# jkw0701/closed_chain_motion_planner

Hardware: AMD Instinct MI355X
Metric: constraint projections/sec (dual-Panda Wine_Bottle) (higher is better)
Workload: dtype f64

## Files before the change

### closed_chain_motion_planner_amd/build.py

```python
import os
import shutil
import subprocess

HERE = os.path.dirname(os.path.abspath(__file__))
CSRC = os.path.join(HERE, "csrc")
LIBDIR = os.path.join(HERE, "lib")
LIBPATH = os.environ.get("CCMP_LIBRARY") or os.path.join(LIBDIR, "libccmp.so")
DEBUG_LIBPATH = os.path.join(LIBDIR, "libccmp_debug.so")
_DEBUG_UNITS = ("ccmp_api.cpp", "ccmp_policy.cpp")
_DEBUG_ONLY_UNITS = [("ccmp_kernels_debug.hip", ["-O3", "-ffp-contract=off", "-DCCMP_USE_FMA", "-DCCMP_LEAN_SQRT", "-DCCMP_LEAN_DIV", "-mllvm", "-disable-machine-licm"])]
ARCH = "gfx950"

_UNITS = [
    ("ccmp_kernels_fd.hip", ["-O3", "-ffp-contract=off", "-DCCMP_USE_FMA", "-DCCMP_LEAN_SQRT", "-DCCMP_ATAN_UNIFORM", "-DCCMP_FD_TI_HOIST",
                             "-mllvm", "-disable-machine-licm", "-mllvm", "-amdgpu-sched-strategy=max-ilp"]
     + os.environ.get("CCMP_FD_EXTRA_FLAGS", "").split()),
    ("ccmp_kernels_wave.hip", ["-O3", "-ffp-contract=off", "-DCCMP_USE_FMA"]),
    ("ccmp_kernels_flat.hip", ["-O3", "-ffp-contract=off", "-DCCMP_USE_FMA", "-mllvm", "-disable-machine-licm", "-mllvm", "-amdgpu-sched-strategy=max-ilp"]),
    ("ccmp_kernels_geo.hip", ["-O3", "-ffp-contract=off", "-DCCMP_USE_FMA", "-mllvm", "-disable-machine-licm", "-mllvm", "-amdgpu-sched-strategy=max-ilp"]),
    ("ccmp_kernels_geo.hip", ["-O3", "-ffp-contract=off", "-DCCMP_USE_FMA", "-DCCMP_GEO_LATENCY", "-DCCMP_SUMS_IN_LANE", "-DCCMP_FLAT_MIN_WAVES=2", "-mllvm", "-amdgpu-sched-strategy=max-ilp"],
     "ccmp_kernels_geo_lat.hip.o"),
    ("ccmp_kernels_geo_scene.hip", ["-O3", "-ffp-contract=off", "-DCCMP_USE_FMA", "-DCCMP_SUMS_IN_LANE", "-DCCMP_FLAT_MIN_WAVES=2", "-mllvm", "-amdgpu-sched-strategy=max-ilp"]),
    ("ccmp_kernels_resident.hip", ["-O3", "-ffp-contract=off", "-DCCMP_USE_FMA", "-DCCMP_SUMS_IN_LANE", "-DCCMP_FLAT_MIN_WAVES=2", "-mllvm", "-amdgpu-sched-strategy=max-ilp"]),
    ("ccmp_kernels_fast.hip", ["-O3", "-ffp-contract=off", "-DCCMP_USE_FMA", "-DCCMP_LEAN_SQRT", "-mllvm", "-disable-machine-licm"]),
    ("ccmp_kernels_scout.hip", ["-O3", "-ffp-contract=fast", "-ffast-math", "-fno-slp-vectorize"]),
    ("ccmp_problem.cpp", ["-O2", "-ffp-contract=off", "-DCCMP_USE_FMA", "-x", "hip"]),
    ("ccmp_api.cpp", ["-O2", "-ffp-contract=off", "-DCCMP_USE_FMA", "-x", "hip"]),
    ("ccmp_policy.cpp", ["-O2", "-x", "hip"]),
    ("ccmp_resident.cpp", ["-O2", "-x", "hip"]),
    ("ccmp_host_io.cpp", ["-O2", "-x", "hip"]),
    ("ccmp_comm.cpp", ["-O2", "-x", "hip"]),
    ("ccmp_kernels_scene.hip", ["-O3", "-ffp-contract=off", "-DCCMP_USE_FMA", "-DCCMP_LEAN_SQRT"]),
    ("ccmp_scene.cpp", ["-O2", "-ffp-contract=off", "-DCCMP_USE_FMA", "-x", "hip"]),
]
_HEADERS = ["ccmp_detmath.h", "ccmp_kin.h", "ccmp_solve.h", "ccmp_fd_common.h", "ccmp_flat_newton.h", "ccmp_host.h", "ccmp_ctx.h", "ccmp_launch.h", "ccmp_policy.h", "ccmp_resident.h", "ccmp_fd_newton_phase1.inc", "ccmp_fd_newton_phase2.inc", "ccmp_geo_edge.h", "ccmp_geo_edge_body.inc", "ccmp_scene.h", "ccmp_clearance.h", "ccmp_row16_eval.inc", "ccmp_row16_step.inc", "ccmp_row16_geo_body.inc", os.path.join("..", "..", "include", "ccmp.h")]


def hipcc_path():
    for cand in (shutil.which("hipcc"), "/opt/rocm/bin/hipcc"):
        if cand and os.path.exists(cand):
            return cand
    raise RuntimeError("hipcc not found: libccmp.so cannot be built (no CPU fallback exists)")


def _stale(target, sources):
    if not os.path.exists(target):
        return True
    t = os.path.getmtime(target)
    return any(os.path.getmtime(s) > t for s in sources if os.path.exists(s))


_SCRATCH_RULES = [
    (r"(project_fd_kernel|project_fd_flat_kernel|project_fd_wave_kernel|geodesic_flat_kernel(_lat)?|geodesic_scene_kernel|geodesic_group_kernel|resident_service_kernel)<(\d+, )?true>", 0),
    (r"(project_fd_kernel|project_fd_flat_kernel|project_fd_wave_kernel|geodesic_flat_kernel(_lat)?|geodesic_scene_kernel|geodesic_group_kernel|resident_service_kernel)<(\d+, )?false>", 136),
    (r"project_pair_kernel|project_row16_kernel", 0),
    (r"geodesic_row16_(scene_)?kernel", 0),
    (r"scout_|clearance", 400),
    (r".", 64),
]


def _demangle(names):
    for tool in ("/opt/rocm/lib/llvm/bin/llvm-cxxfilt", shutil.which("c++filt")):
        if tool and os.path.exists(tool):
            out = subprocess.run([tool], input="\n".join(names), capture_output=True, text=True).stdout.split("\n")
            return dict(zip(names, out))
    return {n: n for n in names}


def parse_resource_remarks(stderr_text):
    import re

    kernels, cur = [], None
    keys = {"TotalSGPRs": "sgprs", "VGPRs": "vgprs", "AGPRs": "agprs", "ScratchSize [bytes/lane]": "scratch", "Occupancy [waves/SIMD]": "occupancy",
            "SGPRs Spill": "sgpr_spill", "VGPRs Spill": "vgpr_spill", "LDS Size [bytes/block]": "lds"}
    for line in stderr_text.splitlines():
        m = re.search(r"remark: (?:\s*)([A-Za-z \[\]/]+): (\S+) \[-Rpass-analysis", line)
        if not m:
            continue
        k, v = m.group(1).strip(), m.group(2)
        if k == "Function Name":
            cur = {"mangled": v}
            kernels.append(cur)
        elif cur is not None and k in keys:
            cur[keys[k]] = int(v)
    dm = _demangle([k["mangled"] for k in kernels])
    for k in kernels:
        k["name"] = dm[k["mangled"]].replace("(anonymous namespace)::", "").split("(")[0].replace("void ", "")
    return kernels


def check_resources(kernels, unit):
    import re

    bad = []
    for k in kernels:
        bound = next(b for rx, b in _SCRATCH_RULES if re.search(rx, k["name"]))
        k["scratch_bound"] = bound
        if k.get("scratch", 0) > bound:
            bad.append("%s: %d B/lane of scratch (bound %d), %d VGPRs, %d spilled" % (k["name"], k["scratch"], bound, k.get("vgprs", -1), k.get("vgpr_spill", -1)))
    if bad and not os.environ.get("CCMP_ALLOW_SPILLS"):
        raise RuntimeError("register allocation of %s regressed (closed_chain_motion_planner_amd/build.py: _SCRATCH_RULES; CCMP_ALLOW_SPILLS=1 "
                           "builds anyway):\n  " % unit + "\n  ".join(bad))


def resource_report():
    import glob
    import json

    return {os.path.basename(f)[:-len(".resources.json")]: json.load(open(f)) for f in sorted(glob.glob(os.path.join(HERE, "build", "*.resources.json")))}


def build_library(force=False, verbose=False):
    os.makedirs(LIBDIR, exist_ok=True)
    objdir = os.path.join(HERE, "build")
    os.makedirs(objdir, exist_ok=True)
    hipcc = hipcc_path()
    headers = [os.path.join(CSRC, h) for h in _HEADERS]
    objs, dbg_objs, jobs = [], [], []
    relink = force
    for src, flags, *obj in _UNITS:
        sp = os.path.join(CSRC, src)
        op = os.path.join(objdir, obj[0] if obj else src + ".o")
        objs.append(op)
        variants = [(op, [])]
        if src in _DEBUG_UNITS:
            dp = os.path.join(objdir, src + ".dbg.o")
            dbg_objs.append(dp)
            variants.append((dp, ["-DCCMP_DEBUG_HOOKS"]))
        else:
            dbg_objs.append(op)
        for target, extra in variants:
            if force or _stale(target, [sp] + headers):
                jobs.append([hipcc, "--offload-arch=" + ARCH, "-fPIC", "-std=c++17"] + flags + extra +
                            (["-Rpass-analysis=kernel-resource-usage"] if src.endswith(".hip") else []) + ["-c", sp, "-o", target])
    for src, flags in _DEBUG_ONLY_UNITS:
        sp, op = os.path.join(CSRC, src), os.path.join(objdir, src + ".o")
        dbg_objs.append(op)
        if force or _stale(op, [sp] + headers):
            jobs.append([hipcc, "--offload-arch=" + ARCH, "-fPIC", "-std=c++17"] + flags + ["-Rpass-analysis=kernel-resource-usage", "-c", sp, "-o", op])
    if jobs:
        import json
        from concurrent.futures import ThreadPoolExecutor

        def run(cmd):
            if verbose:
                print(" ".join(cmd))
            r = subprocess.run(cmd, capture_output=True, text=True)
            rest = "\n".join(ln for ln in r.stderr.splitlines() if "-Rpass-analysis=kernel-resource-usage" not in ln)
            if rest.strip():
                print(rest)
            if r.returncode != 0:
                raise subprocess.CalledProcessError(r.returncode, cmd)
            if "-Rpass-analysis=kernel-resource-usage" in cmd:
                kernels = parse_resource_remarks(r.stderr)
                try:
                    check_resources(kernels, os.path.basename(cmd[-1]))
                except RuntimeError:
                    os.remove(cmd[-1])
                    raise
                json.dump(kernels, open(cmd[-1][:-2] + ".resources.json", "w"), indent=1)

        workers = max(1, min(len(jobs), int(os.environ.get("CCMP_BUILD_JOBS", "0")) or min(4, os.cpu_count() or 1)))
        with ThreadPoolExecutor(workers) as pool:
            list(pool.map(run, jobs))
        relink = True
    default_lib = os.path.join(LIBDIR, "libccmp.so")
    for target, members in ((default_lib, objs), (DEBUG_LIBPATH, dbg_objs)):
        if relink or _stale(target, members):
            cmd = [hipcc, "--offload-arch=" + ARCH, "-shared", "-fPIC", "-o", target] + members
            if verbose:
                print(" ".join(cmd))
            subprocess.run(cmd, check=True)
    return LIBPATH


if __name__ == "__main__":
    print(build_library(force=True, verbose=True))
```

### closed_chain_motion_planner_amd/csrc/ccmp_kernels_fd.hip

```cpp
#include <hip/hip_runtime.h>
#include <stdint.h>

#include "ccmp_fd_common.h"

using namespace ccmp;

namespace {

constexpr int kGroup = 6;
constexpr int kGroupsPerWave = 10;
constexpr int kX = 0;
constexpr int kSC = 14;
constexpr int kPre = 42;
constexpr int kEE = 126;
constexpr int kJ0 = 150;
constexpr int kRec = 165;

#ifndef CCMP_FD_WAVES_PER_SIMD
#define CCMP_FD_WAVES_PER_SIMD 3
#endif
#ifndef CCMP_FD_STOCK_COLUMNS
#define CCMP_FD_STOCK_COLUMNS 1
#endif
#ifndef CCMP_FD_ROWS
#define CCMP_FD_ROWS 1
#endif

template <int ARM, bool STORE, bool STOCK, int I>
__device__ __forceinline__ void chain_at_x_from(const ccmp_consts &K, double *rec, bool writer, double *R, double *o)
{
  if constexpr (I < 7) {
    double Rn[9];
    mulvec_acc_nz<STOCK ? kStockOff[I] : 7>(R, K.offset[ARM][I], o);
    if (STORE && writer) {
#pragma unroll
      for (int k = 0; k < 9; k++) rec[kPre + I * 12 + k] = R[k];
#pragma unroll
      for (int k = 0; k < 3; k++) rec[kPre + I * 12 + 9 + k] = o[k];
    }
    chain_rot<I, STOCK>(K.axis[ARM][I], K.aprod[ARM][I], rec[kSC + 2 * (ARM * 7 + I)], rec[kSC + 2 * (ARM * 7 + I) + 1], R, Rn);
#pragma unroll
    for (int k = 0; k < 9; k++) R[k] = Rn[k];
    chain_at_x_from<ARM, STORE, STOCK, I + 1>(K, rec, writer, R, o);
  }
}
template <int ARM, bool STORE, bool STOCK>
__device__ __forceinline__ void chain_at_x(const ccmp_consts &K, double *rec, bool writer, double *T)
{
  double R[9] = {1, 0, 0, 0, 1, 0, 0, 0, 1}, o[3] = {0, 0, 0};
  if constexpr (STOCK) {
    chain_at_x_from<ARM, STORE, true, 0>(K, rec, writer, R, o);
  } else {
    for (int i = 0; i < 7; i++) {
      double Rj[9], Rn[9];
      mulvec_acc(R, K.offset[ARM][i], o);
      if (STORE && writer) {
#pragma unroll
        for (int k = 0; k < 9; k++) rec[kPre + i * 12 + k] = R[k];
#pragma unroll
        for (int k = 0; k < 3; k++) rec[kPre + i * 12 + 9 + k] = o[k];
      }
      rot_sc(K.axis[ARM][i], K.aprod[ARM][i], rec[kSC + 2 * (ARM * 7 + i)], rec[kSC + 2 * (ARM * 7 + i) + 1], Rj);
      mul33(R, Rj, Rn);
#pragma unroll
      for (int k = 0; k < 9; k++) R[k] = Rn[k];
    }
  }
  tool_pose_t<STOCK>(K, ARM, R, o, &T[0], &T[9]);
}

template <bool TOOL, int I>
__device__ __forceinline__ void chain_rows_from(const ccmp_consts &K, double *rec, const double *sc, int row, bool store,
                                                double &R0, double &R1, double &R2, double &o)
{
  if constexpr (I < 7) {
    constexpr int NZ = kStockOff[I];
    if (NZ & 1) o = CCMP_FMA(R0, K.offset[0][I][0], o);
    if (NZ & 2) o = CCMP_FMA(R1, K.offset[0][I][1], o);
    if (NZ & 4) o = CCMP_FMA(R2, K.offset[0][I][2], o);
    if (store) {
      rec[kPre + I * 12 + 3 * row] = R0;
      rec[kPre + I * 12 + 3 * row + 1] = R1;
      rec[kPre + I * 12 + 3 * row + 2] = R2;
      rec[kPre + I * 12 + 9 + row] = o;
    }
    const double s = sc[2 * I], c = sc[2 * I + 1];
    double n0, n1, n2;
    if constexpr (kStockZ[I] != 0) {
      const double t = 1.0 - c;
      const double w = t + c;
      const double ns = -s;
      n0 = CCMP_FMA(R1, s, R0 * c);
      n1 = CCMP_FMA(R1, c, R0 * ns);
      n2 = R2 * w;
    } else {
      double Rj[9];
      rot_sc(K.axis[0][I], K.aprod[0][I], s, c, Rj);
      n0 = dot3(R0, Rj[0], R1, Rj[3], R2, Rj[6]);
      n1 = dot3(R0, Rj[1], R1, Rj[4], R2, Rj[7]);
      n2 = dot3(R0, Rj[2], R1, Rj[5], R2, Rj[8]);
    }
    R0 = n0; R1 = n1; R2 = n2;
    chain_rows_from<TOOL, I + 1>(K, rec, sc, row, store, R0, R1, R2, o);
  }
}
template <bool TOOL>
__device__ __forceinline__ void chain_rows(const ccmp_consts &K, double *rec, int arm, int row, bool live, int store_arm,
                                           double d_lane, double bp_lane)
{
  double R0 = row == 0 ? 1.0 : 0.0, R1 = row == 1 ? 1.0 : 0.0, R2 = row == 2 ? 1.0 : 0.0, o = 0.0;
  chain_rows_from<TOOL, 0>(K, rec, rec + kSC + 14 * arm, row, live && arm == store_arm, R0, R1, R2, o);
  if constexpr (TOOL) {
    double pf = o;
    if (kStockEe & 1) pf = CCMP_FMA(R0, K.ee[0][0], pf);
    if (kStockEe & 2) pf = CCMP_FMA(R1, K.ee[0][1], pf);
    if (kStockEe & 4) pf = CCMP_FMA(R2, K.ee[0][2], pf);
    const double *Rt = K.R_tool[0];
    const double f0 = dot3(R0, Rt[0], R1, Rt[3], R2, Rt[6]);
    const double f1 = dot3(R0, Rt[1], R1, Rt[4], R2, Rt[7]);
    const double f2 = dot3(R0, Rt[2], R1, Rt[5], R2, Rt[8]);
    if (live) {
      double *T = rec + kEE + 12 * arm;
      T[3 * row] = d_lane * f0;
      T[3 * row + 1] = d_lane * f1;
      T[3 * row + 2] = d_lane * f2;
      T[9 + row] = CCMP_FMA(d_lane, pf, bp_lane);
    }
  }
}

__device__ __forceinline__ void stock_z_step(const ccmp_consts &K, int i, double s, double c, const double *R, double *Rn, double *o)
{
  const double ox = K.offset[0][i][0], oz = K.offset[0][i][2];
#pragma unroll
  for (int r = 0; r < 3; r++) o[r] = CCMP_FMA(R[3 * r + 2], oz, CCMP_FMA(R[3 * r], ox, o[r]));
  mul_zrot(R, s, c, Rn);
}
__device__ __forceinline__ void stock_g_step(const ccmp_consts &K, int i, double s, double c, const double *R, double *Rn, double *o)
{
  const double ox = K.offset[0][i][0];
#pragma unroll
  for (int r = 0; r < 3; r++) o[r] = CCMP_FMA(R[3 * r], ox, o[r]);
  double Rj[9];
  rot_sc(K.axis[0][i], K.aprod[0][i], s, c, Rj);
  mul33(R, Rj, Rn);
}

template <int ARM, bool STOCK>
__device__ __forceinline__ void jacobian_columns(const ccmp_consts &K, double *rec, bool live, int r, bool plus, int nstep)
{
  double To[12];
#pragma unroll
  for (int k = 0; k < 12; k++) To[k] = rec[kEE + (1 - ARM) * 12 + k];
#ifdef CCMP_FD_TI_HOIST
  if (ARM == 0) {
    double ti[3];
    mulTvec(&To[0], &To[9], ti);
#pragma unroll
    for (int k = 0; k < 3; k++) To[9 + k] = ti[k];
  }
#endif
  for (int j = 0; j < 7; j++) {
    const double xj = rec[kX + ARM * 7 + j];
    const double axj = ccmp_abs(xj);
    const double h = 1.4901161193847656e-08 * (axj >= 1 ? axj : 1);
    const double hh = plus ? h : -h;
    double y = xj + hh;
    if (nstep >= 2) y = y + hh;
    if (nstep >= 3) y = y + hh;
    double R[9], o[3], s, c;
#pragma unroll
    for (int k = 0; k < 9; k++) R[k] = rec[kPre + j * 12 + k];
#pragma unroll
    for (int k = 0; k < 3; k++) o[k] = rec[kPre + j * 12 + 9 + k];
    ccmp_sincos(y, &s, &c);
    const double *sc = rec + kSC + 2 * ARM * 7;
    if constexpr (STOCK && CCMP_FD_STOCK_COLUMNS) {
      double Rn[9];
      int i = j + 1;
      if ((j & 1) == 0 && j < 6) {
        const double t = 1.0 - c;
        const double w = t + c;
        const double ns = -s;
#pragma unroll
        for (int rr = 0; rr < 3; rr++) {
          const double a = R[3 * rr], b = R[3 * rr + 1];
          R[3 * rr] = CCMP_FMA(b, s, a * c);
          R[3 * rr + 1] = CCMP_FMA(b, c, a * ns);
          R[3 * rr + 2] = R[3 * rr + 2] * w;
        }
      } else {
        double Rj[9];
        rot_sc(K.axis[0][j], K.aprod[0][j], s, c, Rj);
        mul33(R, Rj, Rn);
        if (j < 6) {
          if (i < 6) stock_z_step(K, i, sc[2 * i], sc[2 * i + 1], Rn, R, o);
          else stock_g_step(K, 6, sc[12], sc[13], Rn, R, o);
          i++;
        } else {
#pragma unroll
          for (int k = 0; k < 9; k++) R[k] = Rn[k];
        }
      }
      for (; i < 5; i += 2) {
        stock_g_step(K, i, sc[2 * i], sc[2 * i + 1], R, Rn, o);
        stock_z_step(K, i + 1, sc[2 * i + 2], sc[2 * i + 3], Rn, R, o);
      }
      if (i == 5) {
        double Rj[9];
        rot_sc(K.axis[0][5], K.aprod[0][5], sc[10], sc[11], Rj);
        mul33(R, Rj, Rn);
        stock_g_step(K, 6, sc[12], sc[13], Rn, R, o);
      }
    } else {
      {
        double Rj[9], Rn[9];
        rot_sc(K.axis[ARM][j], K.aprod[ARM][j], s, c, Rj);
        mul33(R, Rj, Rn);
#pragma unroll
        for (int k = 0; k < 9; k++) R[k] = Rn[k];
      }
      {
        int i = j + 1;
        if ((7 - i) & 1) {
          joint_step(K, ARM, i, sc[2 * i], sc[2 * i + 1], R, o);
          i++;
        }
        for (; i < 7; i += 2) {
          double Rj[9], Rn[9];
          mulvec_acc(R, K.offset[ARM][i], o);
          rot_sc(K.axis[ARM][i], K.aprod[ARM][i], sc[2 * i], sc[2 * i + 1], Rj);
          mul33(R, Rj, Rn);
          mulvec_acc(Rn, K.offset[ARM][i + 1], o);
          rot_sc(K.axis[ARM][i + 1], K.aprod[ARM][i + 1], sc[2 * i + 2], sc[2 * i + 3], Rj);
          mul33(Rn, Rj, R);
        }
      }
    }
#if defined(CCMP_FD_PROBE_MOV) || defined(CCMP_FD_PROBE_FMA)
    {
      int pv = j;
      double pa = xj, pb = xj;
#ifdef CCMP_FD_PROBE_MOV
#pragma unroll
      for (int k = 0; k < CCMP_FD_PROBE_MOV; k++) asm volatile("v_mov_b32 %0, 0x12345678" : "=v"(pv));
#endif
#ifdef CCMP_FD_PROBE_FMA
#pragma unroll
      for (int k = 0; k < CCMP_FD_PROBE_FMA / 2; k++) asm volatile("v_fma_f64 %0, %0, %2, %2\n v_fma_f64 %1, %1, %2, %2" : "+v"(pa), "+v"(pb) : "v"(h));
#endif
      if (pv == 0x7fffffff || pa + pb == 12345.678) rec[kX] = pa;
    }
#endif
    double Tw[12], t[2];
    tool_pose_t<STOCK>(K, ARM, R, o, &Tw[0], &Tw[9]);
#ifdef CCMP_FD_TI_HOIST
    if (ARM == 0) chain_residual_ti(K, &Tw[0], &Tw[9], &To[0], &To[9], t, nullptr, nullptr);
#else
    if (ARM == 0) chain_residual(K, &Tw[0], &Tw[9], &To[0], &To[9], t, nullptr, nullptr);
#endif
    else chain_residual(K, &To[0], &To[9], &Tw[0], &Tw[9], t, nullptr, nullptr);
    if (live) {
      rec[kPre + 12 * j + 2 * r] = t[0];
      rec[kPre + 12 * j + 2 * r + 1] = t[1];
    }
  }
}

template <int ARM>
__device__ __forceinline__ void stencil_combine(double *rec, int r, bool live)
{
#pragma unroll
  for (int n = 0; n < 3; n++) {
    const int e = r + kGroup * n;
    if (e < 14 && live) {
      const int c = e >> 1, row = e & 1;
      const double xj = rec[kX + ARM * 7 + c];
      const double axj = ccmp_abs(xj);
      const double h = 1.4901161193847656e-08 * (axj >= 1 ? axj : 1);
      double y1 = xj, y2 = xj, m[3];
#pragma unroll
      for (int sidx = 0; sidx < 3; sidx++) {
        y1 = y1 + h;
        y2 = y2 - h;
        m[sidx] = (rec[kPre + 12 * c + 2 * sidx + row] - rec[kPre + 12 * c + 2 * (sidx + 3) + row]) / (y1 - y2);
      }
      const double Jv = CCMP_FMA(0.1, m[2], CCMP_FMA(-0.6, m[1], 1.5 * m[0]));
      if (ARM == 0) rec[kJ0 + 2 * c + row] = Jv;
      else rec[kSC + 2 * c + row] = Jv;
    }
  }
}

template <int MODE, bool STOCK>
__global__ __launch_bounds__(64, CCMP_FD_WAVES_PER_SIMD) void project_fd_kernel(
    const ccmp_consts K, const double *__restrict__ q_in, double *__restrict__ q_out, uint8_t *__restrict__ ok_out,
    uint16_t *__restrict__ iters_out, double *__restrict__ q_ambient, unsigned long long B, unsigned long long *queue,
    unsigned long long seed, unsigned long long first_index, double *__restrict__ pool, unsigned long long *pool_count,
    int dump_threshold, const unsigned int *__restrict__ order, const uint16_t *__restrict__ pred, int long_remaining,
    unsigned long long pool_records)
{
  __shared__ double lds[kGroupsPerWave * kRec];
  const int lane = threadIdx.x;
  const int g = lane / kGroup;
  const int r = lane - kGroup * g;
  const bool live = g < kGroupsPerWave;
  const int leader = live ? kGroup * g : 0;
  double *rec = lds + (live ? g : 0) * kRec;
  const bool writer = live && r == 0;
  const bool plus = r < 3;
  const int nstep = (plus ? r : r - 3) + 1;
  const int arm_l = plus ? 0 : 1, row_l = plus ? r : r - 3;
  double d_lane = 0.0, bp_lane = 0.0;
  if constexpr (STOCK) {
    d_lane = arm_l ? (row_l == 0 ? K.base_R[1][0] : (row_l == 1 ? K.base_R[1][4] : K.base_R[1][8]))
                   : (row_l == 0 ? K.base_R[0][0] : (row_l == 1 ? K.base_R[0][4] : K.base_R[0][8]));
    bp_lane = arm_l ? (row_l == 0 ? K.base_p[1][0] : (row_l == 1 ? K.base_p[1][1] : K.base_p[1][2]))
                    : (row_l == 0 ? K.base_p[0][0] : (row_l == 1 ? K.base_p[0][1] : K.base_p[0][2]));
  }

  unsigned long long idx = 0;
  int iter = 0, updates = 0;
  double norm1 = 0.0, norm2 = 0.0;
  bool active = false, drained = false;

  for (;;) {
    {
      const bool want = live && !active && !drained;
      unsigned long long t = 0;
      if (want && r == 0) t = atomicAdd(queue, 1ull);
      t = shfl_u64(t, leader);
      if (want) {
        if (t < B) {
          idx = order ? (unsigned long long)order[t] : t;
          active = true; iter = 0; updates = 0; norm1 = 0.0; norm2 = 0.0;
          if (MODE == 0) {
            const double2 *row = reinterpret_cast<const double2 *>(q_in + idx * 14);
            const double2 a = row[r];
            rec[kX + 2 * r] = a.x;
            rec[kX + 2 * r + 1] = a.y;
            if (r == 0) {
              const double2 b = row[6];
              rec[kX + 12] = b.x;
              rec[kX + 13] = b.y;
            }
          } else {
#pragma unroll
            for (int e = 0; e < 14; e++) {
              if (e % kGroup == r) {
                const double v = ambient_uniform(K, seed, first_index + idx, e);
                if (q_ambient) q_ambient[idx * 14 + e] = v;
                rec[kX + e] = v;
              }
            }
          }
        } else drained = true;
      }
    }
    if (__builtin_amdgcn_ballot_w64(active) == 0ull) break;
    __syncthreads();
    bool dry = __builtin_amdgcn_ballot_w64(drained) != 0ull;
    if (pool != nullptr && !dry) {
      unsigned long long head = 0;
      if (lane == 0) head = __hip_atomic_load(queue, __ATOMIC_RELAXED, __HIP_MEMORY_SCOPE_AGENT);
      head = shfl_u64(head, 0);
      dry = head >= B;
    }
    if (pool != nullptr && dry && dump_threshold > 10) {
      unsigned long long done = 0;
      if (lane == 0) done = __hip_atomic_load(queue + 3, __ATOMIC_RELAXED, __HIP_MEMORY_SCOPE_AGENT);
      done = shfl_u64(done, 0);
      const unsigned long long in_flight = B - done, slots = (unsigned long long)gridDim.x * kGroupsPerWave;
      if (in_flight * 100ull >= slots * (unsigned long long)(dump_threshold - 10)) dry = false;
    }
    if (pool != nullptr && dry &&
        __builtin_popcountll(__builtin_amdgcn_ballot_w64(active && r == 0)) <= dump_threshold) {
      bool is_long = true;
      if (pool_records != 0ull) is_long = active && pred != nullptr && (int)pred[idx] - iter >= long_remaining;
      const unsigned long long mL = __builtin_amdgcn_ballot_w64(active && r == 0 && is_long);
      const unsigned long long mS = __builtin_amdgcn_ballot_w64(active && r == 0 && !is_long);
      unsigned long long bL = 0, bS = 0;
      if (lane == 0) {
        if (mL) bL = atomicAdd(pool_count, (unsigned long long)__builtin_popcountll(mL));
        if (mS) bS = atomicAdd(pool_count + 5, (unsigned long long)__builtin_popcountll(mS));
      }
      bL = shfl_u64(bL, 0);
      bS = shfl_u64(bS, 0);
      const unsigned long long below = (1ull << leader) - 1ull;
      const unsigned long long slot = is_long ? bL + (unsigned long long)__builtin_popcountll(mL & below)
                                              : pool_records - 1ull - (bS + (unsigned long long)__builtin_popcountll(mS & below));
      if (active) {
        double *ent = pool + slot * kPoolEntry;
        for (int e = r; e < 14; e += kGroup) ent[e] = rec[kX + e];
        if (r == 0) {
          ent[14] = __longlong_as_double((long long)idx);
          ent[15] = __hiloint2double(updates, iter);
          ent[16] = norm1;
          ent[17] = norm2;
        }
      }
      break;
    }

#define CCMP_FD_BP bp_lane
#include "ccmp_fd_newton_phase1.inc"
    {
      const bool fin = active && !cont;
      bool bad = false;
      if (fin) {
#pragma unroll
        for (int e = 0; e < 14; e++) {
          if (e % kGroup == r) {
            const double v = rec[kX + e];
            if (v < K.lbe[e % 7]) bad = true;
            if (v > K.ube[e % 7]) bad = true;
          }
        }
        double2 *row = reinterpret_cast<double2 *>(q_out + idx * 14);
        double2 a;
        a.x = rec[kX + 2 * r];
        a.y = rec[kX + 2 * r + 1];
        if (MODE == 1) { a.x = wrap_pi(a.x); a.y = wrap_pi(a.y); }
        row[r] = a;
        if (r == 0) {
          double2 b;
          b.x = rec[kX + 12];
          b.y = rec[kX + 13];
          if (MODE == 1) { b.x = wrap_pi(b.x); b.y = wrap_pi(b.y); }
          row[6] = b;
        }
      }
      const unsigned long long badmask = __builtin_amdgcn_ballot_w64(bad);
      if (fin && r == 0) {
        const bool gbad = ((badmask >> leader) & 0x3Full) != 0ull;
        ok_out[idx] = (uint8_t)((!gbad) && (norm1 < K.tol_pos) && (norm2 < K.tol_rot));
        if (iters_out) iters_out[idx] = (uint16_t)updates;
        if (pool != nullptr && dump_threshold > 10) atomicAdd(queue + 3, 1ull);
      }
      if (fin) active = false;
    }
    if (__builtin_amdgcn_ballot_w64(cont) == 0ull) continue;
    __syncthreads();

#include "ccmp_fd_newton_phase2.inc"
#undef CCMP_FD_BP
  }
}


constexpr int kGPrev = kRec, kGDist = kRec + 14, kGCnt = kRec + 17, kRecG = kRec + 20;
static_assert(kRecG % 2 == 1, "odd record stride: the ten groups stay on distinct LDS banks");

__device__ __forceinline__ double geo_interpolate(double fr, double tg, double tt)
{
  const double pi = 3.14159265358979323846;
  double diff = tg - fr, v;
  if (ccmp_abs(diff) <= pi) v = CCMP_FMA(diff, tt, fr);
  else {
    if (diff > 0.0) diff = 2.0 * pi - diff;
    else diff = -2.0 * pi - diff;
    v = CCMP_FMA(-diff, tt, fr);
    if (v > pi) v -= 2.0 * pi;
    else if (v < -pi) v += 2.0 * pi;
  }
  return v;
}

#ifndef CCMP_GEO_GROUP_WAVES_PER_SIMD
#define CCMP_GEO_GROUP_WAVES_PER_SIMD CCMP_FD_WAVES_PER_SIMD
#endif
template <bool STOCK>
__global__ __launch_bounds__(64, CCMP_GEO_GROUP_WAVES_PER_SIMD) void geodesic_group_kernel(
    const ccmp_consts K, const double delta, const double lambda, const double *__restrict__ from, const double *__restrict__ to,
    unsigned long long E, int max_states, double *__restrict__ states, int *__restrict__ n_states, uint8_t *__restrict__ ok_out,
    int *__restrict__ newton_iters, unsigned long long *queue, const unsigned int *__restrict__ order,
    double *__restrict__ carry_out, int round_budget, double *__restrict__ pool, unsigned long long *pool_count, int handover_pct,
    const uint8_t *__restrict__ target_ok)
{
  __shared__ double lds[kGroupsPerWave * kRecG];
  __shared__ double lane_bp[64];
  const int lane = threadIdx.x;
  const int g = lane / kGroup;
  const int r = lane - kGroup * g;
  const bool live = g < kGroupsPerWave;
  const int leader = live ? kGroup * g : 0;
  double *rec = lds + (live ? g : 0) * kRecG;
  const bool writer = live && r == 0;
  const bool plus = r < 3;
  const int nstep = (plus ? r : r - 3) + 1;
  const int arm_l = plus ? 0 : 1, row_l = plus ? r : r - 3;
  double d_lane = 0.0, bp_lane = 0.0;
  if constexpr (STOCK) {
    d_lane = arm_l ? (row_l == 0 ? K.base_R[1][0] : (row_l == 1 ? K.base_R[1][4] : K.base_R[1][8]))
                   : (row_l == 0 ? K.base_R[0][0] : (row_l == 1 ? K.base_R[0][4] : K.base_R[0][8]));
    bp_lane = arm_l ? (row_l == 0 ? K.base_p[1][0] : (row_l == 1 ? K.base_p[1][1] : K.base_p[1][2]))
                    : (row_l == 0 ? K.base_p[0][0] : (row_l == 1 ? K.base_p[0][1] : K.base_p[0][2]));
  }
  lane_bp[lane] = bp_lane;
#ifndef CCMP_GEO_GROUP_OPAQUE
#define CCMP_GEO_GROUP_OPAQUE 1
#endif
  auto lane_opaque = [](int v) {
#if CCMP_GEO_GROUP_OPAQUE
    asm volatile("" : "+v"(v));
#endif
    return v;
  };

  unsigned long long edge = 0;
  int iter = 0, updates = 0;
  double norm1 = 0.0, norm2 = 0.0;
  bool active = false, drained = false;

  for (;;) {
    {
      const bool want = live && !active && !drained;
      unsigned long long t = 0;
      if (want && r == 0) t = atomicAdd(queue, 1ull);
      t = shfl_u64(t, leader);
      if (want) {
        if (t < E) {
          edge = order ? (unsigned long long)order[t] : t;
          const double *fr = from + edge * 14ull, *tg = to + edge * 14ull;
          double *out = states + edge * (unsigned long long)max_states * 14ull;
          double acc = 0.0;
#pragma unroll
          for (int i = 0; i < 14; i++) {
            const double diff = fr[i] - tg[i];
            acc = CCMP_FMA(diff, diff, acc);
          }
          const double dist = ccmp_sqrt(acc);
          const double total = 0.0, maxd = dist * lambda;
          const bool tgt = target_ok == nullptr || target_ok[edge] != 0;
          const bool enter = tgt && dist > delta;
          const double tt = delta / dist;
          for (int e = lane_opaque(r); e < 14; e += kGroup) {
            const double a = fr[e];
            rec[kGPrev + e] = a;
            if (max_states > 0) out[e] = a;
            if (enter) rec[kX + e] = geo_interpolate(a, tg[e], tt);
          }
          if (r == 0) {
            rec[kGDist] = dist;
            rec[kGDist + 1] = total;
            rec[kGDist + 2] = maxd;
            int *cnt = reinterpret_cast<int *>(rec + kGCnt);
            cnt[0] = 1; cnt[1] = 0; cnt[2] = 0;
          }
          if (enter) {
            active = true; iter = 0; updates = 0; norm1 = 0.0; norm2 = 0.0;
          } else if (r == 0) {
            n_states[edge] = 1;
            ok_out[edge] = (uint8_t)(tgt && dist <= delta);
            if (newton_iters) newton_iters[edge] = 0;
            if (carry_out) { carry_out[2ull * edge] = total; carry_out[2ull * edge + 1ull] = maxd; }
            if (pool) atomicAdd(queue + 3, 1ull);
          }
        } else drained = true;
      }
    }
    if (__builtin_amdgcn_ballot_w64(active) == 0ull) {
      if (__builtin_amdgcn_ballot_w64(live && !drained) == 0ull) break;
      continue;
    }
    __syncthreads();
    if (pool != nullptr) {
      unsigned long long head = 0, fin_count = 0;
      if (lane == 0) {
        head = __hip_atomic_load(queue, __ATOMIC_RELAXED, __HIP_MEMORY_SCOPE_AGENT);
        fin_count = __hip_atomic_load(queue + 3, __ATOMIC_RELAXED, __HIP_MEMORY_SCOPE_AGENT);
      }
      head = shfl_u64(head, 0);
      fin_count = shfl_u64(fin_count, 0);
      const unsigned long long in_flight = E - fin_count, slots = (unsigned long long)gridDim.x * kGroupsPerWave;
      if (head >= E && in_flight * 100ull < slots * (unsigned long long)handover_pct) {
        const unsigned long long m = __builtin_amdgcn_ballot_w64(active && r == 0);
        unsigned long long base = 0;
        if (lane == 0 && m) base = atomicAdd(pool_count, (unsigned long long)__builtin_popcountll(m));
        base = shfl_u64(base, 0);
        if (active) {
          double *ent = pool + (base + (unsigned long long)__builtin_popcountll(m & ((1ull << lane_opaque(leader)) - 1ull))) * (unsigned long long)kGeoPoolEntry;
          for (int e = lane_opaque(r); e < 14; e += kGroup) { ent[e] = rec[kX + e]; ent[14 + e] = rec[kGPrev + e]; }
          if (r == 0) {
            const int *cnt = reinterpret_cast<const int *>(rec + kGCnt);
            ent[28] = rec[kGDist]; ent[29] = rec[kGDist + 1]; ent[30] = rec[kGDist + 2];
            ent[31] = __longlong_as_double((long long)edge);
            ent[32] = __hiloint2double(cnt[0], cnt[1]);
            ent[33] = __hiloint2double(cnt[2], iter);
            ent[34] = __hiloint2double(0, updates);
            ent[35] = norm1; ent[36] = norm2;
          }
        }
        break;
      }
    }

#define CCMP_FD_BP lane_bp[lane_opaque(lane)]
#include "ccmp_fd_newton_phase1.inc"
    {
      const bool fin = active && !cont;
      bool bad = false;
      if (fin) {
#pragma unroll
        for (int e = 0; e < 14; e++) {
          if (e % kGroup == r) {
            const double v = rec[kX + e];
            if (v < K.lbe[e % 7]) bad = true;
            if (v > K.ube[e % 7]) bad = true;
          }
        }
      }
      const unsigned long long badmask = __builtin_amdgcn_ballot_w64(bad);
      if (fin) {
        const bool jv = ((badmask >> leader) & 0x3Full) == 0ull;
        const bool conv = (norm1 < K.tol_pos) && (norm2 < K.tol_rot);
        int *cnt = reinterpret_cast<int *>(rec + kGCnt);
        int n = cnt[0], its = cnt[1] + updates;
        const int rounds = cnt[2] + updates + 1;
        double dist = rec[kGDist], total = rec[kGDist + 1];
        const double maxd = rec[kGDist + 2];
        const double *tg = to + edge * 14ull;
        double *out = states + edge * (unsigned long long)max_states * 14ull;
        double s_acc = 0.0, d_acc = 0.0;
#pragma unroll
        for (int i = 0; i < 14; i++) {
          const double xi = rec[kX + i];
          const double ds = rec[kGPrev + i] - xi, dd = xi - tg[i];
          s_acc = CCMP_FMA(ds, ds, s_acc);
          d_acc = CCMP_FMA(dd, dd, d_acc);
        }
        bool done = true, fits = true, suspended = false;
        do {
          if (!(conv && jv)) break;
          const double step = ccmp_sqrt(s_acc), newDist = ccmp_sqrt(d_acc);
          double delta_o = delta;
          asm volatile("" : "+v"(delta_o));
          if (step > lambda * delta_o) break;
          const double total_before = total;
          total += step;
          if (total > maxd) break;
          if (newDist >= dist) break;
          if (n >= max_states) { fits = false; n = max_states + 1; total = total_before; its -= updates; break; }
          dist = newDist;
          for (int e = lane_opaque(r); e < 14; e += kGroup) out[(unsigned long long)n * 14ull + e] = rec[kX + e];
          n++;
          if (!(dist >= delta)) break;
          if (round_budget > 0 && rounds >= round_budget) { suspended = true; break; }
          done = false;
        } while (0);
        if (done) {
          if (r == 0) {
            n_states[edge] = n;
            ok_out[edge] = suspended ? (uint8_t)2 : (uint8_t)(fits && dist <= delta);
            if (newton_iters) newton_iters[edge] = its;
            if (carry_out) { carry_out[2ull * edge] = total; carry_out[2ull * edge + 1ull] = maxd; }
            if (pool) atomicAdd(queue + 3, 1ull);
          }
          active = false;
        } else {
          const double tt = delta / dist;
          for (int e = lane_opaque(r); e < 14; e += kGroup) {
            const double a = rec[kX + e];
            rec[kGPrev + e] = a;
            rec[kX + e] = geo_interpolate(a, tg[e], tt);
          }
          if (r == 0) {
            cnt[0] = n; cnt[1] = its; cnt[2] = rounds;
            rec[kGDist] = dist;
            rec[kGDist + 1] = total;
          }
          iter = 0; updates = 0; norm1 = 0.0; norm2 = 0.0;
        }
      }
    }
    if (__builtin_amdgcn_ballot_w64(cont) == 0ull) continue;
    __syncthreads();

#include "ccmp_fd_newton_phase2.inc"
#undef CCMP_FD_BP
  }
}


__global__ void clear_words_kernel(unsigned int *__restrict__ w, unsigned int n)
{
  const unsigned int i = blockIdx.x * blockDim.x + threadIdx.x;
  if (i < n) w[i] = 0u;
}

__device__ __forceinline__ void publish_done(unsigned int *done_flag, unsigned int done_seq)
{
  if (done_flag != nullptr) {
    __threadfence_system();
    __hip_atomic_store(done_flag, done_seq, __ATOMIC_RELEASE, __HIP_MEMORY_SCOPE_SYSTEM);
  }
}

__global__ __launch_bounds__(64) void function_kernel(const ccmp_consts K, const double *__restrict__ q, double *__restrict__ f, size_t B,
                                                      unsigned int *done_flag, unsigned int done_seq)
{
  size_t i = (size_t)blockIdx.x * blockDim.x + threadIdx.x;
  if (i >= B) return;
  double x[14], out[2];
#pragma unroll
  for (int e = 0; e < 14; e++) x[e] = q[i * 14 + e];
  residual(K, x, out);
  f[2 * i] = out[0];
  f[2 * i + 1] = out[1];
  publish_done(done_flag, done_seq);
}

__global__ __launch_bounds__(64) void is_satisfied_kernel(const ccmp_consts K, const double *__restrict__ q, uint8_t *__restrict__ ok, size_t B,
                                                          unsigned int *done_flag, unsigned int done_seq)
{
  size_t i = (size_t)blockIdx.x * blockDim.x + threadIdx.x;
  if (i >= B) return;
  double x[14], f[2];
#pragma unroll
  for (int e = 0; e < 14; e++) x[e] = q[i * 14 + e];
  residual(K, x, f);
  const bool finite = (f[0] - f[0] == 0.0) && (f[1] - f[1] == 0.0);
  ok[i] = (uint8_t)(finite && f[0] <= K.tol_pos && f[1] <= K.tol_rot);
  publish_done(done_flag, done_seq);
}

__global__ void joint_valid_kernel(const ccmp_consts K, const double *__restrict__ q, uint8_t *__restrict__ ok, size_t B,
                                   unsigned int *done_flag, unsigned int done_seq)
{
  size_t i = (size_t)blockIdx.x * blockDim.x + threadIdx.x;
  if (i >= B) return;
  bool good = true;
  for (int e = 0; e < 14; e++) {
    const double v = q[i * 14 + e];
    const int jj = e < 7 ? e : e - 7;
    if (v < K.lbe[jj]) good = false;
    if (v > K.ube[jj]) good = false;
  }
  ok[i] = (uint8_t)good;
  publish_done(done_flag, done_seq);
}

__global__ void ambient_uniform_kernel(const ccmp_consts K, unsigned long long seed, unsigned long long first,
                                       double *__restrict__ q, size_t n )
{
  size_t t = (size_t)blockIdx.x * blockDim.x + threadIdx.x;
  if (t >= n) return;
  q[t] = ambient_uniform(K, seed, first + t / 14, (int)(t % 14));
}

__global__ void ambient_near_kernel(const ccmp_consts K, unsigned long long seed, unsigned long long first,
                                    const double *__restrict__ ref, int ref_stride, double dist, double *__restrict__ q, size_t n)
{
  size_t t = (size_t)blockIdx.x * blockDim.x + threadIdx.x;
  if (t >= n) return;
  const size_t i = t / 14;
  const int j = (int)(t % 14);
  q[t] = ambient_near(K, seed, first + i, j, ref[i * (size_t)ref_stride + j], dist);
}
__global__ void ambient_gaussian_kernel(const ccmp_consts K, unsigned long long seed, unsigned long long first,
                                        const double *__restrict__ ref, int ref_stride, double stddev, double *__restrict__ q,
                                        size_t n)
{
  size_t t = (size_t)blockIdx.x * blockDim.x + threadIdx.x;
  if (t >= n) return;
  const size_t i = t / 14;
  const int j = (int)(t % 14);
  q[t] = ambient_gaussian(K, seed, first + i, j, ref[i * (size_t)ref_stride + j], stddev);
}

__global__ __launch_bounds__(64) void t_wo_kernel(const ccmp_consts K, const double *__restrict__ q, int q_stride, double *__restrict__ out, size_t B)
{
  size_t i = (size_t)blockIdx.x * blockDim.x + threadIdx.x;
  if (i >= B) return;
  double x[7], Rw[9], pw[3], R[9], p[3];
#pragma unroll
  for (int e = 0; e < 7; e++) x[e] = q[i * (size_t)q_stride + e];
  fk_arm(K, 0, x, Rw, pw);
  mul33(Rw, K.t_o7i_R, R);
  p[0] = pw[0]; p[1] = pw[1]; p[2] = pw[2];
  mulvec_acc(Rw, K.t_o7i_p, p);
#pragma unroll
  for (int k = 0; k < 9; k++) out[i * 12 + k] = R[k];
#pragma unroll
  for (int k = 0; k < 3; k++) out[i * 12 + 9 + k] = p[k];
}

__global__ void enforce_bounds_kernel(double *__restrict__ q, size_t n)
{
  size_t t = (size_t)blockIdx.x * blockDim.x + threadIdx.x;
  if (t >= n) return;
  q[t] = wrap_pi(q[t]);
}

__global__ void compact_count_kernel(const uint8_t *__restrict__ ok, size_t B, unsigned int *__restrict__ block_counts)
{
  __shared__ unsigned int wsum[4];
  size_t i = (size_t)blockIdx.x * 256 + threadIdx.x;
  const bool v = i < B && ok[i] != 0;
  const unsigned long long m = __builtin_amdgcn_ballot_w64(v);
  if ((threadIdx.x & 63) == 0) wsum[threadIdx.x >> 6] = (unsigned)__builtin_popcountll(m);
  __syncthreads();
  if (threadIdx.x == 0) block_counts[blockIdx.x] = wsum[0] + wsum[1] + wsum[2] + wsum[3];
}
__global__ void compact_scan_kernel(unsigned int *__restrict__ block_counts, size_t nblocks,
                                    unsigned long long *__restrict__ total)
{
  __shared__ unsigned long long part[1024];
  const size_t per = (nblocks + 1023) / 1024;
  const size_t lo = (size_t)threadIdx.x * per, hi = lo + per < nblocks ? lo + per : nblocks;
  unsigned long long s = 0;
  for (size_t k = lo; k < hi; k++) s += block_counts[k];
  part[threadIdx.x] = s;
  __syncthreads();
  if (threadIdx.x == 0) {
    unsigned long long run = 0;
    for (int k = 0; k < 1024; k++) { unsigned long long v = part[k]; part[k] = run; run += v; }
    *total = run;
  }
  __syncthreads();
  unsigned long long run = part[threadIdx.x];
  for (size_t k = lo; k < hi; k++) { unsigned int v = block_counts[k]; block_counts[k] = (unsigned int)run; run += v; }
}
__global__ void compact_scatter_kernel(const double *__restrict__ q, const uint8_t *__restrict__ ok, size_t B,
                                       const unsigned int *__restrict__ block_offsets, double *__restrict__ out,
                                       size_t capacity)
{
  __shared__ unsigned int wsum[4];
  size_t i = (size_t)blockIdx.x * 256 + threadIdx.x;
  const bool v = i < B && ok[i] != 0;
  const unsigned long long m = __builtin_amdgcn_ballot_w64(v);
  const int lane = threadIdx.x & 63, w = threadIdx.x >> 6;
  if (lane == 0) wsum[w] = (unsigned)__builtin_popcountll(m);
  __syncthreads();
  unsigned int base = block_offsets[blockIdx.x];
  for (int k = 0; k < w; k++) base += wsum[k];
  if (v) {
    const unsigned int pos = base + (unsigned)__builtin_popcountll(m & ((1ull << lane) - 1ull));
    if (pos < capacity) {
#pragma unroll
      for (int e = 0; e < 14; e++) out[(size_t)pos * 14 + e] = q[i * 14 + e];
    }
  }
}

}

namespace ccmp_launch {

hipError_t geodesic_group(const GeoCall &g, int blocks, unsigned long long *queue, const unsigned int *order, double *pool,
                          unsigned long long *pool_count, int handover_pct, const uint8_t *target_ok, hipStream_t st)
{
  if (g.K->stock && g.K->twin_arms)
    hipLaunchKernelGGL(geodesic_group_kernel<true>, dim3(blocks), dim3(64), 0, st, *g.K, g.delta, g.lambda, g.from, g.to, (unsigned long long)g.E,
                       g.max_states, g.states, g.n_states, g.ok, g.newton_iters, queue, order, g.carry_out, g.round_budget, pool, pool_count, handover_pct, target_ok);
  else
    hipLaunchKernelGGL(geodesic_group_kernel<false>, dim3(blocks), dim3(64), 0, st, *g.K, g.delta, g.lambda, g.from, g.to, (unsigned long long)g.E,
                       g.max_states, g.states, g.n_states, g.ok, g.newton_iters, queue, order, g.carry_out, g.round_budget, pool, pool_count, handover_pct, target_ok);
  return hipGetLastError();
}

hipError_t clear_words(void *words, size_t n_u32, hipStream_t st)
{
  hipLaunchKernelGGL(clear_words_kernel, dim3((unsigned)((n_u32 + 255) / 256)), dim3(256), 0, st, (unsigned int *)words, (unsigned int)n_u32);
  return hipGetLastError();
}

hipError_t project_group(const ProjectCall &c, int blocks, unsigned long long *queue, double *pool, int dump_threshold,
                         const unsigned int *order, const uint16_t *pred, int long_remaining, size_t pool_records, hipStream_t st)
{
#define CCMP_LAUNCH_GROUP(MODE, STOCK)                                                                                                    \
  hipLaunchKernelGGL((project_fd_kernel<MODE, STOCK>), dim3(blocks), dim3(64), 0, st, *c.K, c.q_in, c.q_out, c.ok, c.iters, c.q_ambient, \
                     (unsigned long long)c.B, queue + kQTicket, c.seed, c.first, pool, queue + kQPool, dump_threshold, order, pred,       \
                     long_remaining, (unsigned long long)pool_records)
  if (c.mode == 0) {
    if (c.K->stock && c.K->twin_arms) CCMP_LAUNCH_GROUP(0, true);
    else CCMP_LAUNCH_GROUP(0, false);
  } else {
    if (!(c.K->stock && c.K->twin_arms)) return hipErrorInvalidValue;
    CCMP_LAUNCH_GROUP(1, true);
  }
#undef CCMP_LAUNCH_GROUP
  return hipGetLastError();
}

hipError_t function(const ccmp_consts *K, const double *q, double *f, size_t B, unsigned int *done_flag, unsigned int done_seq, hipStream_t st)
{
  if (B != 1) done_flag = nullptr;
  hipLaunchKernelGGL(function_kernel, dim3((unsigned)((B + 63) / 64)), dim3(64), 0, st, *K, q, f, B, done_flag, done_seq);
  return hipGetLastError();
}
hipError_t is_satisfied(const ccmp_consts *K, const double *q, uint8_t *ok, size_t B, unsigned int *done_flag, unsigned int done_seq,
                        hipStream_t st)
{
  if (B != 1) done_flag = nullptr;
  hipLaunchKernelGGL(is_satisfied_kernel, dim3((unsigned)((B + 63) / 64)), dim3(64), 0, st, *K, q, ok, B, done_flag, done_seq);
  return hipGetLastError();
}
hipError_t joint_valid(const ccmp_consts *K, const double *q, uint8_t *ok, size_t B, unsigned int *done_flag, unsigned int done_seq,
                       hipStream_t st)
{
  if (B != 1) done_flag = nullptr;
  hipLaunchKernelGGL(joint_valid_kernel, dim3((unsigned)((B + 255) / 256)), dim3(256), 0, st, *K, q, ok, B, done_flag, done_seq);
  return hipGetLastError();
}
hipError_t ambient_uniform(const ccmp_consts *K, unsigned long long seed, unsigned long long first, double *q, size_t B, hipStream_t st)
{
  size_t n = B * 14;
  hipLaunchKernelGGL(ambient_uniform_kernel, dim3((unsigned)((n + 255) / 256)), dim3(256), 0, st, *K, seed, first, q, n);
  return hipGetLastError();
}
hipError_t ambient_ref(const ccmp_consts *K, int kind, unsigned long long seed, unsigned long long first, const double *ref, int ref_stride,
                       double param, double *q, size_t B, hipStream_t st)
{
  size_t n = B * 14;
  if (kind == 0)
    hipLaunchKernelGGL(ambient_near_kernel, dim3((unsigned)((n + 255) / 256)), dim3(256), 0, st, *K, seed, first, ref,
                       ref_stride, param, q, n);
  else
    hipLaunchKernelGGL(ambient_gaussian_kernel, dim3((unsigned)((n + 255) / 256)), dim3(256), 0, st, *K, seed, first, ref,
                       ref_stride, param, q, n);
  return hipGetLastError();
}
hipError_t t_wo(const ccmp_consts *K, const double *q, int q_stride, double *out, size_t B, hipStream_t st)
{
  hipLaunchKernelGGL(t_wo_kernel, dim3((unsigned)((B + 63) / 64)), dim3(64), 0, st, *K, q, q_stride, out, B);
  return hipGetLastError();
}
hipError_t enforce_bounds(double *q, size_t B, hipStream_t st)
{
  size_t n = B * 14;
  hipLaunchKernelGGL(enforce_bounds_kernel, dim3((unsigned)((n + 255) / 256)), dim3(256), 0, st, q, n);
  return hipGetLastError();
}
hipError_t compact(const double *q, const uint8_t *ok, size_t B, double *out, size_t capacity, unsigned int *block_counts,
                   unsigned long long *total, hipStream_t st)
{
  const size_t nblocks = (B + 255) / 256;
  hipLaunchKernelGGL(compact_count_kernel, dim3((unsigned)nblocks), dim3(256), 0, st, ok, B, block_counts);
  hipLaunchKernelGGL(compact_scan_kernel, dim3(1), dim3(1024), 0, st, block_counts, nblocks, total);
  hipLaunchKernelGGL(compact_scatter_kernel, dim3((unsigned)nblocks), dim3(256), 0, st, q, ok, B, block_counts, out, capacity);
  return hipGetLastError();
}

}
```

Measured before the change: 16.51 million.

## Share fixed-joint rotation matrices across group lanes via LDS in FD Jacobian

Before the finite-difference Jacobian column loop, the per-joint rotation matrices for joints 3, 5 and 6 (whose angles are not perturbed by later columns) are computed once. Lanes r==0..2 write them into otherwise dead slots of the per-group LDS record. The stock column path then reads these matrices from LDS instead of recomputing rot_sc for every column. This removes redundant rotation construction at the cost of two extra __syncthreads and LDS traffic. Opaque asm barriers on row/leader are added to steer the compiler's scheduling.

```diff
diff --git a/closed_chain_motion_planner_amd/build.py b/closed_chain_motion_planner_amd/build.py
--- a/closed_chain_motion_planner_amd/build.py
+++ b/closed_chain_motion_planner_amd/build.py
@@ -12,7 +12,7 @@
 ARCH = "gfx950"
 
 _UNITS = [
-    ("ccmp_kernels_fd.hip", ["-O3", "-ffp-contract=off", "-DCCMP_USE_FMA", "-DCCMP_LEAN_SQRT", "-DCCMP_ATAN_UNIFORM", "-DCCMP_FD_TI_HOIST",
+    ("ccmp_kernels_fd.hip", ["-O3", "-ffp-contract=off", "-DCCMP_USE_FMA", "-DCCMP_LEAN_SQRT", "-DCCMP_ATAN_UNIFORM", "-DCCMP_FD_TI_HOIST", "-DCCMP_FD_SHARE_ROT",
                              "-mllvm", "-disable-machine-licm", "-mllvm", "-amdgpu-sched-strategy=max-ilp"]
      + os.environ.get("CCMP_FD_EXTRA_FLAGS", "").split()),
     ("ccmp_kernels_wave.hip", ["-O3", "-ffp-contract=off", "-DCCMP_USE_FMA"]),
diff --git a/closed_chain_motion_planner_amd/csrc/ccmp_kernels_fd.hip b/closed_chain_motion_planner_amd/csrc/ccmp_kernels_fd.hip
--- a/closed_chain_motion_planner_amd/csrc/ccmp_kernels_fd.hip
+++ b/closed_chain_motion_planner_amd/csrc/ccmp_kernels_fd.hip
@@ -109,7 +109,13 @@
                                            double d_lane, double bp_lane)
 {
   double R0 = row == 0 ? 1.0 : 0.0, R1 = row == 1 ? 1.0 : 0.0, R2 = row == 2 ? 1.0 : 0.0, o = 0.0;
+#ifdef CCMP_FD_SHARE_ROT
+  int row_st = row;
+  asm volatile("" : "+v"(row_st));
+  chain_rows_from<TOOL, 0>(K, rec, rec + kSC + 14 * arm, row_st, live && arm == store_arm, R0, R1, R2, o);
+#else
   chain_rows_from<TOOL, 0>(K, rec, rec + kSC + 14 * arm, row, live && arm == store_arm, R0, R1, R2, o);
+#endif
   if constexpr (TOOL) {
     double pf = o;
     if (kStockEe & 1) pf = CCMP_FMA(R0, K.ee[0][0], pf);
@@ -146,6 +152,41 @@
   mul33(R, Rj, Rn);
 }
 
+#ifdef CCMP_FD_SHARE_ROT
+template <int ARM>
+__device__ __forceinline__ constexpr int rot_slot(int m)
+{
+  return ARM == 0 ? kEE + 12 + 9 * m : (m < 2 ? kEE + 9 * m : kSC);
+}
+static_assert(rot_slot<0>(2) + 9 == kRec && rot_slot<1>(1) + 9 <= kEE + 24 && rot_slot<1>(2) + 9 <= kSC + 14, "rotation matrices inside the dead slots");
+__device__ __forceinline__ void stock_g_step_shared(const ccmp_consts &K, int i, const double *Rj_lds, const double *R, double *Rn, double *o)
+{
+  const double ox = K.offset[0][i][0];
+#pragma unroll
+  for (int r = 0; r < 3; r++) o[r] = CCMP_FMA(R[3 * r], ox, o[r]);
+  double Rj[9];
+#pragma unroll
+  for (int k = 0; k < 9; k++) Rj[k] = Rj_lds[k];
+  mul33(R, Rj, Rn);
+}
+__device__ __forceinline__ void stock_g_step_kept(const ccmp_consts &K, int i, bool kept, const double *Rj_lds, const double *sc, const double *R,
+                                                  double *Rn, double *o)
+{
+  const double ox = K.offset[0][i][0];
+#pragma unroll
+  for (int r = 0; r < 3; r++) o[r] = CCMP_FMA(R[3 * r], ox, o[r]);
+  double Rj[9];
+  if (kept) {
+#pragma unroll
+    for (int k = 0; k < 9; k++) Rj[k] = Rj_lds[k];
+    mul33(R, Rj, Rn);
+  } else {
+    rot_sc(K.axis[0][i], K.aprod[0][i], sc[2 * i], sc[2 * i + 1], Rj);
+    mul33(R, Rj, Rn);
+  }
+}
+#endif
+
 template <int ARM, bool STOCK>
 __device__ __forceinline__ void jacobian_columns(const ccmp_consts &K, double *rec, bool live, int r, bool plus, int nstep)
 {
@@ -158,6 +199,23 @@
     mulTvec(&To[0], &To[9], ti);
 #pragma unroll
     for (int k = 0; k < 3; k++) To[9 + k] = ti[k];
+  }
+#endif
+#ifdef CCMP_FD_SHARE_ROT
+  if constexpr (STOCK && CCMP_FD_STOCK_COLUMNS) {
+    __syncthreads();
+#pragma unroll
+    for (int m = 0; m < 3; m++) {
+      constexpr int kJoint[3] = {3, 5, 6};
+      const int jm = kJoint[m];
+      double Rj[9];
+      rot_sc(K.axis[0][jm], K.aprod[0][jm], rec[kSC + 2 * (ARM * 7 + jm)], rec[kSC + 2 * (ARM * 7 + jm) + 1], Rj);
+      if (live && r == m) {
+#pragma unroll
+        for (int k = 0; k < 9; k++) rec[rot_slot<ARM>(m) + k] = Rj[k];
+      }
+    }
+    __syncthreads();
   }
 #endif
   for (int j = 0; j < 7; j++) {
@@ -195,13 +253,30 @@
         mul33(R, Rj, Rn);
         if (j < 6) {
           if (i < 6) stock_z_step(K, i, sc[2 * i], sc[2 * i + 1], Rn, R, o);
+#ifdef CCMP_FD_SHARE_ROT
+          else stock_g_step_shared(K, 6, rec + rot_slot<ARM>(2), Rn, R, o);
+#else
           else stock_g_step(K, 6, sc[12], sc[13], Rn, R, o);
+#endif
           i++;
         } else {
 #pragma unroll
           for (int k = 0; k < 9; k++) R[k] = Rn[k];
         }
       }
+#ifdef CCMP_FD_SHARE_ROT
+      for (; i < 5; i += 2) {
+        stock_g_step_kept(K, i, i == 3, rec + rot_slot<ARM>(0), sc, R, Rn, o);
+        stock_z_step(K, i + 1, sc[2 * i + 2], sc[2 * i + 3], Rn, R, o);
+      }
+      if (i == 5) {
+        double Rj[9];
+#pragma unroll
+        for (int k = 0; k < 9; k++) Rj[k] = rec[rot_slot<ARM>(1) + k];
+        mul33(R, Rj, Rn);
+        stock_g_step_shared(K, 6, rec + rot_slot<ARM>(2), Rn, R, o);
+      }
+#else
       for (; i < 5; i += 2) {
         stock_g_step(K, i, sc[2 * i], sc[2 * i + 1], R, Rn, o);
         stock_z_step(K, i + 1, sc[2 * i + 2], sc[2 * i + 3], Rn, R, o);
@@ -212,6 +287,7 @@
         mul33(R, Rj, Rn);
         stock_g_step(K, 6, sc[12], sc[13], Rn, R, o);
       }
+#endif
     } else {
       {
         double Rj[9], Rn[9];
@@ -612,7 +688,11 @@
       }
       const unsigned long long badmask = __builtin_amdgcn_ballot_w64(bad);
       if (fin) {
+#ifdef CCMP_FD_SHARE_ROT
+        const bool jv = ((badmask >> (STOCK ? lane_opaque(leader) : leader)) & 0x3Full) == 0ull;
+#else
         const bool jv = ((badmask >> leader) & 0x3Full) == 0ull;
+#endif
         const bool conv = (norm1 < K.tol_pos) && (norm2 < K.tol_rot);
         int *cnt = reinterpret_cast<int *>(rec + kGCnt);
         int n = cnt[0], its = cnt[1] + updates;
```

After: 16.74 million (median of 6 runs). +1.4%, better.
